# bupt-ai-cz/HIAST

Measured on AMD Instinct MI355X. Metric: self-training images/sec (fwd+bwd+pseudo-label) at 1024x512, higher is better.
Workload: dtype fp16

## Files before the change

hiast_amd/_lib.py:

```python
import ctypes
import os

import torch

_HERE = os.path.dirname(os.path.abspath(__file__))
LIB_PATH = os.environ.get("HIAST_LIB") or os.path.join(_HERE, "csrc", "libhiast_hip.so")

c_int, c_i64, c_f32, c_sz, c_vp = (ctypes.c_int, ctypes.c_int64, ctypes.c_float, ctypes.c_size_t,
                                   ctypes.c_void_p)

SIGNATURES = {
    "hiast_version": (c_int, []),
    "hiast_error_string": (ctypes.c_char_p, [c_int]),
    "hiast_upsample_bilinear_ac_fwd": (c_int, [c_vp, c_vp] + [c_int] * 6 + [c_vp]),
    "hiast_upsample_bilinear_ac_bwd": (c_int, [c_vp, c_vp] + [c_int] * 6 + [c_vp]),
    "hiast_plabel_pass1_workspace_bytes": (c_sz, [c_int]),
    "hiast_plabel_pass1": (c_int, [c_vp] + [c_int] * 6 + [c_vp, c_vp, c_vp, c_vp, c_sz, c_vp]),
    "hiast_plabel_pass2": (c_int, [c_vp, c_vp, c_vp, c_int, c_int, c_i64, c_vp, c_vp, c_vp, c_vp]),
    "hiast_plabel_strided_hist_workspace_bytes": (c_sz, [c_i64, c_int]),
    "hiast_plabel_strided_hist": (c_int, [c_vp, c_vp, c_i64, c_int, c_int, c_vp, c_vp, c_vp, c_vp, c_sz, c_vp]),
    "hiast_tta_fused": (c_int, [c_vp] * 6 + [c_int] * 5 + [c_vp, c_vp, c_vp]),
    "hiast_dinput_fwd": (c_int, [c_vp, c_int, c_vp] + [c_int] * 6 + [c_vp]),
    "hiast_dinput_bwd": (c_int, [c_vp, c_int, c_vp, c_vp, c_vp] + [c_int] * 6 + [c_vp]),
    "hiast_st_loss_workspace_bytes": (c_sz, [c_int] * 6),
# ... 30 lines not shown
    "hiast_stream_destroy": (c_int, [c_vp]),
    "hiast_igemm_stats_rows": (c_int, [c_i64, c_int, c_int, c_int, c_int]),
    "hiast_igemm_dgrad_bn_stats": (c_int, [c_vp, c_vp, c_vp] + [c_int] * 7 + [c_vp] * 6 + [c_int, c_int, c_vp]),
    "hiast_xconv_dgrad_gated_bn_stats_rows": (c_int, [c_i64, c_int, c_int]),
    "hiast_xconv_dgrad_gated_bn_stats": (c_int, [c_vp] * 10 + [c_i64, c_int, c_int, c_int, c_vp]),
    "hiast_igemm_dgrad_s2": (c_int, [c_vp, c_vp, c_vp] + [c_int] * 6 + [c_vp]),
    "hiast_igemm_dgrad_bn_stats_rows": (c_int, [c_i64, c_int, c_int, c_int]),
    "hiast_bn_nhwc_stats_from_partial": (c_int, [c_vp, c_int, c_int, c_vp, c_vp]),
    "hiast_conv_wgrad_workspace_bytes": (c_sz, [c_int] * 6),
    "hiast_conv_wgrad_nhwc": (c_int, [c_vp, c_vp, c_vp] + [c_int] * 9 + [c_vp, c_sz, c_vp]),
    "hiast_conv_wgrad_group_workspace_bytes": (c_sz, [c_vp, c_int]),
    "hiast_conv_wgrad_group_nhwc": (c_int, [c_vp, c_int, c_int, c_vp, c_sz, c_vp]),
    "hiast_conv_wgrad_small_workspace_bytes": (c_sz, [c_int] * 6),
    "hiast_conv_wgrad_small_nhwc": (c_int, [c_vp, c_vp, c_vp] + [c_int] * 9 + [c_vp, c_sz, c_vp]),
    "hiast_pack_conv_weight": (c_int, [c_vp, c_int, c_int, c_int, c_int, c_int, c_vp, c_vp, c_vp]),
    "hiast_bn_nhwc_workspace_bytes": (c_sz, [c_int]),
    "hiast_bn_nhwc_stats": (c_int, [c_vp, c_i64, c_int, c_vp, c_vp, c_sz, c_int, c_vp]),
    "hiast_bn_nhwc_apply": (c_int, [c_vp] * 8 + [ctypes.c_double, c_f32, c_f32, c_int, c_vp, c_vp, c_i64, c_int, c_vp,
                                    c_int, c_vp]),
    "hiast_bn_nhwc_apply_partial": (c_int, [c_vp] * 8 + [c_int, ctypes.c_double, c_f32, c_f32, c_int, c_vp, c_vp, c_i64,
                                            c_int, c_vp, c_int, c_vp]),
    "hiast_bn_nhwc_bwd_stats": (c_int, [c_vp] * 7 + [c_int, c_i64, c_int, c_vp, c_vp, c_sz, c_int, c_vp]),
    "hiast_bn_nhwc_bwd_apply": (c_int, [c_vp] * 8 + [ctypes.c_double, c_int, c_vp, c_vp, c_vp, c_vp, c_i64, c_int, c_int,
                                        c_vp]),
    "hiast_pack_conv_weight_multi": (c_int, [c_vp, c_vp, c_vp, c_int, c_int, c_vp]),
    "hiast_split_planes": (c_int, [c_vp, c_vp, c_i64, c_int, c_int, c_vp]),
    "hiast_stem_tail": (c_int, [c_vp, c_int, c_vp, c_vp, c_vp, c_vp, c_f32, c_vp, c_int, c_int, c_int, c_int, c_int, c_vp]),
    "hiast_stem_eval": (c_int, [c_vp] * 6 + [c_f32, c_vp, c_int, c_int, c_int, c_int, c_vp]),
    "hiast_stem_train_blocks": (c_int, [c_int] * 3),
    "hiast_stem_train_fwd": (c_int, [c_vp, c_vp, c_vp, c_vp, c_int, c_int, c_int, c_int, c_vp]),
    "hiast_stem_wgrad_workspace_bytes": (c_sz, [c_int] * 3),
    "hiast_stem_wgrad": (c_int, [c_vp, c_vp, c_vp, c_int, c_int, c_int, c_int, c_vp, c_sz, c_vp]),
    "hiast_ema_update": (c_int, [c_vp, c_vp, c_vp, c_int, c_f32, c_f32, c_vp]),
    "hiast_normalize_u8": (c_int, [c_vp, c_vp, c_int, c_i64, c_vp, c_vp, c_vp]),
    "hiast_maxpool3x3s2_nhwc_fwd": (c_int, [c_vp, c_vp, c_vp, c_int, c_int, c_int, c_int, c_int, c_vp]),
    "hiast_maxpool3x3s2_nhwc_bwd": (c_int, [c_vp, c_vp, c_vp, c_int, c_int, c_int, c_int, c_int, c_vp]),
    "hiast_multi_copy": (c_int, [c_vp, c_int, c_vp]),
    "hiast_aug_geometry_u8": (c_int, [c_vp] * 6 + [c_int] * 4 + [c_vp]),
    "hiast_aug_hist_u8": (c_int, [c_vp] * 5 + [c_int, c_i64, c_vp]),
    "hiast_aug_colour_u8": (c_int, [c_vp] * 5 + [c_int, c_i64, c_vp]),
    "hiast_aug2_table_u8": (c_int, [c_vp] * 6 + [c_int, c_i64, c_vp]),
    "hiast_aug2_colour_u8": (c_int, [c_vp] * 6 + [c_int, c_i64, c_vp]),
    "hiast_aug2_blur_u8": (c_int, [c_vp] * 5 + [c_int] * 3 + [c_vp]),
    "hiast_adam_prepare": (c_int, [c_vp, c_vp, c_vp, c_vp]),
    "hiast_adam_step": (c_int, [c_vp, c_vp, c_vp, c_int, ctypes.c_double, ctypes.c_double, c_f32, c_f32, c_vp, c_vp]),
    "hiast_disc_conv_workspace_bytes": (c_sz, [c_int] * 5),
    "hiast_disc_conv_fwd": (c_int, [c_vp] * 4 + [c_int] * 6 + [c_vp]),
    "hiast_disc_conv_dgrad": (c_int, [c_vp] * 4 + [c_int] * 6 + [c_vp, c_sz, c_vp]),
    "hiast_disc_conv_wgrad": (c_int, [c_vp] * 5 + [c_int] * 6 + [c_vp, c_sz, c_vp]),
    "hiast_confusion_hist": (c_int, [c_vp, c_vp, c_i64, c_int, c_vp, c_vp, c_vp, c_vp]),
}



class WgradJob(ctypes.Structure):
    _fields_ = [("dy", c_vp), ("x", c_vp), ("dw", c_vp)] + [(n, ctypes.c_int32) for n in
                                                             ("B", "H", "W", "Cin", "Cout", "taps", "stride", "dil")]


NBINS = 15361
PROB_FX_SHIFT = 30
IGNORE = 255

_lib = None


# ... 43 lines not shown
```

hiast_amd/csrc/igemm.hip:

```cpp
#include "igemm_kernel.h"

namespace hiast {

template <int PL>
__device__ __forceinline__ size_t ig_wp_elem(int n, int t, int k, int taps, int KO)
{
    const size_t row = ((size_t)n * taps + t) * PL * KO;
    return PL == 2 ? row + (size_t)(k >> 5) * 64 + (k & 31) : row + k;
}

template <int PL, bool F16 = false>
__global__ __launch_bounds__(256) void pack_conv_weight_kernel(const float* __restrict__ w,
                                                               unsigned short* __restrict__ wp,
                                                               unsigned short* __restrict__ wpt, int N, int K, int taps,
                                                               int mode)
{
    const long long idx = (long long)blockIdx.x * 256 + threadIdx.x;
    if (idx >= (long long)N * taps * K) return;
    const int k = (int)(idx % K);
    const int t = (int)((idx / K) % taps);
    const int n = (int)(idx / ((long long)K * taps));
    const float v = w[((size_t)n * K + k) * taps + t];
    unsigned short h, l = 0;
    if (F16) h = H16<true>::enc(v);
// ... 46 lines not shown
                if (PL == 2) *reinterpret_cast<uint4*>(d + 32) = *reinterpret_cast<const uint4*>(&lo[nt * PK_PITCH + c * 8]);
            }
        }
        if (adj) {
            for (int e = threadIdx.x; e < 64 * taps * (TN / 8); e += 256) {
                const int c = e % (TN / 8), kt = e / (TN / 8);
                const int k = kt / taps, t = kt - k * taps;
                unsigned short vh[8], vl[8];
#pragma unroll
                for (int j = 0; j < 8; ++j) {
                    vh[j] = hi[((c * 8 + j) * taps + t) * PK_PITCH + k];
                    if (PL == 2) vl[j] = lo[((c * 8 + j) * taps + t) * PK_PITCH + k];
                }
                unsigned short* d = adj + ig_wp_elem<PL>(k0 + k, taps - 1 - t, n0 + nh + c * 8, taps, N);
                *reinterpret_cast<uint4*>(d) = make_uint4(vh[0] | (unsigned)vh[1] << 16, vh[2] | (unsigned)vh[3] << 16,
                                                          vh[4] | (unsigned)vh[5] << 16, vh[6] | (unsigned)vh[7] << 16);
                if (PL == 2)
                    *reinterpret_cast<uint4*>(d + 32) = make_uint4(vl[0] | (unsigned)vl[1] << 16, vl[2] | (unsigned)vl[3] << 16,
                                                                   vl[4] | (unsigned)vl[5] << 16, vl[6] | (unsigned)vl[7] << 16);
            }
        }
    }
}

template <int PL, bool F16 = false>
__global__ __launch_bounds__(256) void pack_conv_weight_tiled_kernel(const float* __restrict__ w,
                                                                     unsigned short* __restrict__ wp,
                                                                     unsigned short* __restrict__ wpt, int N, int K,
                                                                     int taps, int mode)
{
    extern __shared__ __attribute__((aligned(16))) unsigned short lds[];
    const int kt = K / 64;
    pack_tile<PL, F16>(w, wp, wpt, N, K, taps, mode, (int)(blockIdx.x / kt) * 64, (int)(blockIdx.x % kt) * 64, lds);
}

__global__ __launch_bounds__(256) void pack_conv_weight_multi_kernel(const hiast_pack_rec* __restrict__ table,
                                                                     const int32_t* __restrict__ chunk_tensor,
                                                                     const int64_t* __restrict__ chunk_start)
{
    extern __shared__ __attribute__((aligned(16))) unsigned short lds[];
    const hiast_pack_rec r = table[chunk_tensor[blockIdx.x]];
    const int kt = r.K / 64;
    const int tile = (int)chunk_start[blockIdx.x];
    const int n0 = (tile / kt) * 64, k0 = (tile % kt) * 64;
    if (r.planes == HIAST_FMT_SPLIT_BF16)
        pack_tile<2>(r.w, (unsigned short*)r.wp, (unsigned short*)r.wpt, r.N, r.K, r.taps, r.mode, n0, k0, lds);
    else if (r.planes == HIAST_FMT_FP16)
        pack_tile<1, true>(r.w, (unsigned short*)r.wp, (unsigned short*)r.wpt, r.N, r.K, r.taps, r.mode, n0, k0, lds);
    else
        pack_tile<1>(r.w, (unsigned short*)r.wp, (unsigned short*)r.wpt, r.N, r.K, r.taps, r.mode, n0, k0, lds);
}

__global__ __launch_bounds__(256) void to_planes_kernel(const float* __restrict__ x, unsigned short* __restrict__ p,
                                                        long long M, int C)
{
    const long long total8 = M * C / 8;
    for (long long i = (long long)blockIdx.x * 256 + threadIdx.x; i < total8; i += (long long)gridDim.x * 256) {
        const long long m = (i * 8) / C;
        const int c = (int)((i * 8) - m * C);
        const float4 a = reinterpret_cast<const float4*>(x)[2 * i], b = reinterpret_cast<const float4*>(x)[2 * i + 1];
        const float v[8] = {a.x, a.y, a.z, a.w, b.x, b.y, b.z, b.w};
        unsigned ph[4], pl_[4];
#pragma unroll
        for (int q = 0; q < 4; ++q) {
            unsigned short h0, l0, h1, l1;
            ig_split(v[2 * q], h0, l0);
// ... 365 lines not shown
    else if (dtype == 1) { if (planes == 2) L(1, 2); else L(1, 1); }
    else { if (planes == 2) L(0, 2); else L(0, 1); }
#undef LF
#undef L
    HIAST_CHECK_LAUNCH();
    return 0;
}

extern "C" int hiast_split_planes(float* x, void* planes, int64_t M, int C, int inverse, hiast_stream_t stream)
{
    if (!x || !planes) return HIAST_E_ARG;
    if (M <= 0 || C <= 0) return HIAST_E_ARG;
    if (C % 32 != 0 || ((((uintptr_t)x) | ((uintptr_t)planes)) & 15)) return HIAST_E_RANGE;
    const long long total8 = (long long)M * C / 8;
    long long nb = (total8 + 255) / 256;
    const int grid = (int)(nb < 1 ? 1 : (nb > 8192 ? 8192 : nb));
    if (inverse)
        hipLaunchKernelGGL(hiast::from_planes_kernel, dim3(grid), dim3(256), 0, (hipStream_t)stream,
                           (const unsigned short*)planes, x, (long long)M, C);
    else
        hipLaunchKernelGGL(hiast::to_planes_kernel, dim3(grid), dim3(256), 0, (hipStream_t)stream, (const float*)x,
                           (unsigned short*)planes, (long long)M, C);
    HIAST_CHECK_LAUNCH();
    return 0;
}

extern "C" int hiast_pack_conv_weight_multi(const hiast_pack_rec* table, const int32_t* chunk_tensor,
                                            const int64_t* chunk_start, int n_chunks, int max_taps, hiast_stream_t stream)
{
    if (!table || !chunk_tensor || !chunk_start) return HIAST_E_ARG;
    if (n_chunks <= 0 || max_taps <= 0) return HIAST_E_ARG;
    if (max_taps > 9) return HIAST_E_RANGE;
    const size_t lds_bytes = (size_t)32 * max_taps * hiast::PK_PITCH * sizeof(unsigned short);
    hipLaunchKernelGGL(hiast::pack_conv_weight_multi_kernel, dim3(n_chunks), dim3(256), lds_bytes, (hipStream_t)stream, table,
                       chunk_tensor, chunk_start);
    HIAST_CHECK_LAUNCH();
    return 0;
}
```

hiast_amd/csrc/misc.hip:

```cpp
#include <hip/hip_bf16.h>

#include <atomic>

#include "common.h"

namespace hiast {

__global__ __launch_bounds__(256) void ema_kernel(const hiast_ema_rec* __restrict__ table,
                                                  const int32_t* __restrict__ chunk_tensor,
                                                  const int64_t* __restrict__ chunk_start,
                                                  float gamma, float omg)
{
    const hiast_ema_rec r = table[chunk_tensor[blockIdx.x]];
    const int64_t s = chunk_start[blockIdx.x];
    const int64_t e = (s + 65536 < r.n) ? s + 65536 : r.n;
    float* __restrict__ d = r.ema;
    const float* __restrict__ p = r.p;
    const bool vec = ((((uintptr_t)d) | ((uintptr_t)p)) & 15) == 0;
    if (vec) {
        const int64_t nv = (e - s) / 4;
        float4* d4 = reinterpret_cast<float4*>(d + s);
        const float4* p4 = reinterpret_cast<const float4*>(p + s);
        for (int64_t i = threadIdx.x; i < nv; i += 256) {
            float4 a = d4[i], b = p4[i];
            a.x = a.x * gamma + b.x * omg;
            a.y = a.y * gamma + b.y * omg;
            a.z = a.z * gamma + b.z * omg;
            a.w = a.w * gamma + b.w * omg;
            d4[i] = a;
        }
        for (int64_t i = s + nv * 4 + threadIdx.x; i < e; i += 256) d[i] = d[i] * gamma + p[i] * omg;
    } else {
        for (int64_t i = s + threadIdx.x; i < e; i += 256) d[i] = d[i] * gamma + p[i] * omg;
    }
}

__global__ __launch_bounds__(256) void normalize_u8_kernel(const unsigned char* __restrict__ img, float* __restrict__ out,
                                                           long long HW, float m0, float m1, float m2, float s0, float s1,
                                                           float s2)
{
    const int b = blockIdx.y;
    const unsigned char* src = img + (size_t)b * HW * 3;
    float* dst = out + (size_t)b * 3 * HW;
    for (long long p = (long long)blockIdx.x * 256 + threadIdx.x; p < HW; p += (long long)gridDim.x * 256) {
        const float r = (float)src[p * 3] / 255.0f, g = (float)src[p * 3 + 1] / 255.0f, bl = (float)src[p * 3 + 2] / 255.0f;
        dst[p] = (r - m0) / s0;
        dst[HW + p] = (g - m1) / s1;
        dst[2 * HW + p] = (bl - m2) / s2;
    }
}

__global__ __launch_bounds__(256) void multi_copy_kernel(const hiast_copy_rec* __restrict__ table)
{
    const hiast_copy_rec r = table[blockIdx.x];
    unsigned char* d = (unsigned char*)r.dst;
    const unsigned char* s = (const unsigned char*)r.src;
    if (((((uintptr_t)d) | ((uintptr_t)s)) & 15) == 0) {
        const int64_t nv = r.nbytes / 16;
        for (int64_t i = threadIdx.x; i < nv; i += 256) reinterpret_cast<uint4*>(d)[i] = reinterpret_cast<const uint4*>(s)[i];
        for (int64_t i = nv * 16 + threadIdx.x; i < r.nbytes; i += 256) d[i] = s[i];
    } else {
        for (int64_t i = threadIdx.x; i < r.nbytes; i += 256) d[i] = s[i];
    }
}

__global__ void adam_prepare_kernel(hiast_adam_ctl* __restrict__ ctl, const float* __restrict__ grad_scale,
                                    const float* __restrict__ found_inf)
// ... 148 lines not shown
    return 0;
}
extern "C" int hiast_stream_destroy(hiast_stream_t s)
{
    if (!s) return HIAST_E_ARG;
    const hipError_t e = hipStreamDestroy((hipStream_t)s);
    if (e != hipSuccess) { (void)hipGetLastError(); return (int)e; }
    return 0;
}

extern "C" const char* hiast_error_string(int code)
{
    switch (code) {
        case 0: return "ok";
        case HIAST_E_ARG: return "hiast: null pointer or non-positive extent";
        case HIAST_E_RANGE: return "hiast: extent outside the range the kernels are built for";
        case HIAST_E_WS: return "hiast: workspace too small";
        default: return code > 0 ? hipGetErrorString((hipError_t)code) : "hiast: unknown error";
    }
}

extern "C" int hiast_ema_update(const hiast_ema_rec* table, const int32_t* chunk_tensor,
                                const int64_t* chunk_start, int n_chunks, float gamma,
                                float one_minus_gamma, hiast_stream_t stream)
{
    if (!table || !chunk_tensor || !chunk_start) return HIAST_E_ARG;
    if (n_chunks <= 0) return HIAST_E_ARG;
    hipLaunchKernelGGL(hiast::ema_kernel, dim3(n_chunks), dim3(256), 0, (hipStream_t)stream, table,
                       chunk_tensor, chunk_start, gamma, one_minus_gamma);
    HIAST_CHECK_LAUNCH();
    return 0;
}

extern "C" int hiast_confusion_hist(const int64_t* pred, const int64_t* target, int64_t N, int K,
                                    int64_t* inter, int64_t* area_pred, int64_t* area_tgt,
                                    hiast_stream_t stream)
{
    if (!pred || !target || !inter || !area_pred || !area_tgt) return HIAST_E_ARG;
    if (N <= 0 || K <= 0) return HIAST_E_ARG;
    if (K > 1024) return HIAST_E_RANGE;
    int64_t nb = (N + 256 * 16 - 1) / (256 * 16);
    int grid = (int)(nb < 1 ? 1 : (nb > 2048 ? 2048 : nb));
    hipLaunchKernelGGL(hiast::confusion_kernel, dim3(grid), dim3(256), 3 * K * sizeof(unsigned),
                       (hipStream_t)stream, pred, target, N, K, (unsigned long long*)inter,
                       (unsigned long long*)area_pred, (unsigned long long*)area_tgt);
    HIAST_CHECK_LAUNCH();
    return 0;
}

extern "C" int hiast_adam_step(const hiast_adam_rec* table, const int32_t* chunk_tensor, const int64_t* chunk_start,
                               int n_chunks, double beta1, double beta2, float eps, float weight_decay,
                               const hiast_adam_ctl* ctl, hiast_stream_t stream)
{
    if (!table || !chunk_tensor || !chunk_start) return HIAST_E_ARG;
    if (n_chunks <= 0) return HIAST_E_ARG;
    hipLaunchKernelGGL(hiast::adam_kernel, dim3(n_chunks), dim3(256), 0, (hipStream_t)stream, table, chunk_tensor,
                       chunk_start, (float)beta1, (float)beta2, (float)(1.0 - beta1), (float)(1.0 - beta2), eps,
                       weight_decay, ctl, beta1, beta2);
    HIAST_CHECK_LAUNCH();
    return 0;
}

extern "C" int hiast_adam_prepare(hiast_adam_ctl* ctl, const float* grad_scale, const float* found_inf,
                                  hiast_stream_t stream)
{
    if (!ctl) return HIAST_E_ARG;
// ... 170 lines not shown
```

hiast_amd/kernels.py:

```python
import ctypes

import numpy as np
import torch

from . import _lib
from . import switches as _SW
from ._lib import NBINS, check


def _stream():
    return ctypes.c_void_p(torch._C._cuda_getCurrentRawStream(torch._C._cuda_getDevice()))


def _ptr(t):
    return ctypes.c_void_p(t.data_ptr()) if t is not None else ctypes.c_void_p(0)


def h2d_async(host, device, out=None):
    stage = torch.from_numpy(np.ascontiguousarray(host)).pin_memory()
    if out is None:
        return stage.to(device, non_blocking=True)
    out.copy_(stage.view(out.dtype).reshape(out.shape) if stage.dtype != out.dtype else stage.reshape(out.shape),
              non_blocking=True)
    return out
# ... 485 lines not shown
    def __init__(self, ema_tensors, src_tensors):
        assert len(ema_tensors) == len(src_tensors) and len(ema_tensors) > 0
        dev = ema_tensors[0].device
        recs = np.zeros((len(ema_tensors), 3), dtype=np.int64)
        ct, cs = [], []
        for i, (e, p) in enumerate(zip(ema_tensors, src_tensors)):
            _req(e, torch.float32, None, "ema tensor")
            _req(p, torch.float32, None, "student tensor")
            assert e.numel() == p.numel()
            recs[i] = (e.data_ptr(), p.data_ptr(), e.numel())
            for s in range(0, e.numel(), self.CHUNK):
                ct.append(i)
                cs.append(s)
        self.keep = (list(ema_tensors), list(src_tensors))
        self.table = torch.from_numpy(recs).to(dev)
        self.chunk_tensor = torch.tensor(ct, dtype=torch.int32, device=dev)
        self.chunk_start = torch.tensor(cs, dtype=torch.int64, device=dev)
        self.n_chunks = len(ct)
        self.ptrs = recs[:, :2].copy()

    def still_valid(self):
        return all(e.data_ptr() == a and p.data_ptr() == b
                   for (e, p, (a, b)) in zip(self.keep[0], self.keep[1], self.ptrs))

    def matches(self, ema_tensors, src_tensors):
        return len(ema_tensors) == len(self.ptrs) and all(
            e.data_ptr() == a and p.data_ptr() == b for (e, p, (a, b)) in zip(ema_tensors, src_tensors, self.ptrs))


def ema_update(plan, gamma):
    check(_lib.load().hiast_ema_update(_ptr(plan.table), _ptr(plan.chunk_tensor), _ptr(plan.chunk_start),
                                       plan.n_chunks, float(np.float32(gamma)), float(np.float32(1 - gamma)),
                                       _stream()), "hiast_ema_update")


def normalize_u8(img_u8, mean, std):
    _req(img_u8, torch.uint8, 4, "img_u8")
    B, H, W, three = img_u8.shape
    assert three == 3 and len(mean) == 3 and len(std) == 3
    out = torch.empty((B, 3, H, W), dtype=torch.float32, device=img_u8.device)
    m = (ctypes.c_float * 3)(*[float(v) for v in mean])
    s_ = (ctypes.c_float * 3)(*[float(v) for v in std])
    if B:
        check(_lib.load().hiast_normalize_u8(_ptr(img_u8), _ptr(out), B, H * W, m, s_, _stream()), "hiast_normalize_u8")
    return out


class CopyPlan:

    def __init__(self, dsts, srcs):
        assert len(dsts) == len(srcs) and len(dsts) > 0
        recs = np.zeros((len(dsts), 3), dtype=np.int64)
        for i, (d, s_) in enumerate(zip(dsts, srcs)):
            if not (d.is_cuda and s_.is_cuda and d.is_contiguous() and s_.is_contiguous() and d.dtype == s_.dtype
                    and d.numel() == s_.numel()):
                raise ValueError("multi_copy: tensor %d: contiguous HIP tensors of equal dtype and size required" % i)
            recs[i] = (d.data_ptr(), s_.data_ptr(), d.numel() * d.element_size())
        self.keep = (list(dsts), list(srcs))
        self.ptrs = recs[:, :2].copy()
        self.table = torch.from_numpy(recs).to(dsts[0].device)
        self.n = len(dsts)

    def still_valid(self):
        return all(d.data_ptr() == a and s_.data_ptr() == b for (d, s_, (a, b)) in zip(self.keep[0], self.keep[1], self.ptrs))

    def matches(self, dsts, srcs):
# ... 476 lines not shown
    M, C2 = p.shape
    x = torch.empty((M, C2 // 2), dtype=torch.float32, device=p.device)
    check(_lib.load().hiast_split_planes(_ptr(x), _ptr(p), M, C2 // 2, 1, _stream()), "hiast_split_planes")
    return x


def pack_conv_weight(weight, fmt, transpose=False, both=False):
    fmt = int(fmt)
    planes, h16 = (2 if fmt == FMT_SPLIT_BF16 else 1), fmt_dtype(fmt)
    w = weight.detach()
    if w.dim() == 2:
        w = w.reshape(w.shape[0], w.shape[1], 1, 1)
    _req(w, torch.float32, 4, "weight")
    N, K_, kh, kw = w.shape
    fwd_shape, adj_shape = (N, kh * kw, planes * K_), (K_, kh * kw, planes * N)
    wpt = None
    if both:
        wp = torch.empty(fwd_shape, dtype=h16, device=w.device)
        wpt = torch.empty(adj_shape, dtype=h16, device=w.device)
        mode = 2
    else:
        wp = torch.empty(adj_shape if transpose else fwd_shape, dtype=h16, device=w.device)
        mode = 1 if transpose else 0
    check(_lib.load().hiast_pack_conv_weight(_ptr(w), N, K_, kh * kw, fmt, mode, _ptr(wp), _ptr(wpt), _stream()),
          "hiast_pack_conv_weight")
    return (wp, wpt) if both else wp


class PackPlan:
    CHUNK = 65536
    REC = np.dtype([("w", np.int64), ("wp", np.int64), ("wpt", np.int64), ("N", np.int32), ("K", np.int32),
                    ("taps", np.int32), ("planes", np.int32), ("mode", np.int32), ("pad", np.int32)])

    def __init__(self, weights, fmt, adjoint):
        assert len(weights) > 0 and len(weights) == len(adjoint)
        dev = weights[0].device
        fmt = int(fmt)
        planes, h16 = (2 if fmt == FMT_SPLIT_BF16 else 1), fmt_dtype(fmt)
        self.weights, self.fmt = list(weights), fmt
        self.wp, self.wpt = [], []
        host = np.zeros(len(weights), dtype=self.REC)
        lists = {}
        for i, (w, adj) in enumerate(zip(weights, adjoint)):
            _req(w.detach(), torch.float32, 4, "weight")
            N, K_, kh, kw = w.shape
            taps = kh * kw
            wp = torch.empty((N, taps, planes * K_), dtype=h16, device=dev)
            wpt = torch.empty((K_, taps, planes * N), dtype=h16, device=dev) if adj else None
            self.wp.append(wp)
            self.wpt.append(wpt)
            host[i] = (w.data_ptr(), wp.data_ptr(), wpt.data_ptr() if adj else 0, N, K_, taps, fmt, 2 if adj else 0, 0)
            if N % 64 or K_ % 64 or taps > 9:
                raise ValueError("PackPlan: channel counts must be multiples of 64 (got %d x %d)" % (N, K_))
            ct, cs = lists.setdefault(taps, ([], []))
            for tile in range((N // 64) * (K_ // 64)):
                ct.append(i)
                cs.append(tile)
        self.ptrs = [w.data_ptr() for w in weights]
        self.table = torch.from_numpy(host.view(np.uint8).reshape(-1).copy()).to(dev)
        self.launches = [(taps, torch.tensor(ct, dtype=torch.int32, device=dev), torch.tensor(cs, dtype=torch.int64, device=dev),
                          len(ct)) for taps, (ct, cs) in sorted(lists.items())]
        self.versions = None

    def still_valid(self):
        return all(w.data_ptr() == p for w, p in zip(self.weights, self.ptrs))

    def refresh(self):
        v = [w._version for w in self.weights]
        if v == self.versions:
            return False
        for taps, ct, cs, n in self.launches:
            check(_lib.load().hiast_pack_conv_weight_multi(_ptr(self.table), _ptr(ct), _ptr(cs), n, taps, _stream()),
                  "hiast_pack_conv_weight_multi")
        self.versions = v
        return True


def igemm_bn_act(x, wp, planes, bn, res, relu, stride=1, dil=1, out_f32=False, want_stats=False, res_gate=None):
    _req16(x, 4, "x")
    PL = 2 if int(planes) == 2 else 1
    fmt = fmt_of(x, PL)
# ... 393 lines not shown
```

hiast_amd/workflows/trainer/base_trainer.py:

```python
import os

import numpy as np
import torch
import torch.distributed as dist

from hiast_amd import functional as HF
from torch.nn.parallel import DistributedDataParallel as DDP
from torch.utils.data import DataLoader, DistributedSampler

from hiast_amd.sseg.datasets import utils as du
from hiast_amd.utils import comm, metrics, utils
from hiast_amd.utils.registry.registries import DATASET
from hiast_amd.utils.result_recorder import ResultRecorder


def autocast_dtype(cfg):
    if cfg.train.apex_opt == "O0":
        return None
    kind = getattr(cfg.train, "amp_dtype", "fp16")
    if kind not in ("bf16", "fp16"):
        raise ValueError("train.amp_dtype must be 'bf16' or 'fp16', got %r" % (kind,))
    return torch.bfloat16 if kind == "bf16" else torch.float16


def make_grad_scaler(amp_dtype):
    if amp_dtype is torch.float16:
        return torch.amp.GradScaler("cuda", init_scale=2.0 ** 16, growth_factor=2.0, backoff_factor=0.5, growth_interval=2000)
    return None


def _worker_init(_worker_id):
    try:
        os.nice(10)
    except OSError:
        pass


class _EpochChain(torch.utils.data.Sampler):

    def __init__(self, sampler, batch_size, drop_last):
        self.sampler, self.batch_size, self.drop_last = sampler, batch_size, drop_last

    def __iter__(self):
        while True:
            n = 0
            for b in torch.utils.data.BatchSampler(self.sampler, self.batch_size, self.drop_last):
                n += 1
                yield b
            if n == 0:
                return
            self.sampler.set_epoch(self.sampler.epoch + 1)

    def __len__(self):
        return len(torch.utils.data.BatchSampler(self.sampler, self.batch_size, self.drop_last))


class _Bare(torch.nn.Module):

    def __init__(self, m):
        super().__init__()
# ... 240 lines not shown
```

include/hiast_hip.h:

```cpp
#ifndef HIAST_HIP_H
#define HIAST_HIP_H

#include <stddef.h>
#include <stdint.h>

#ifdef __cplusplus
extern "C" {
#endif

#define HIAST_ABI_VERSION 6

#define HIAST_E_ARG   (-1)
#define HIAST_E_RANGE (-2)
#define HIAST_E_WS    (-3)

#define HIAST_NBINS 15361
#define HIAST_PROB_FX_SHIFT 30
#define HIAST_MAX_CLASSES 32
#define HIAST_FMT_BF16 1
#define HIAST_FMT_SPLIT_BF16 2
#define HIAST_FMT_FP16 3
#define HIAST_IGNORE 255

typedef void* hiast_stream_t;
// ... 145 lines not shown
size_t hiast_conv_wgrad_group_workspace_bytes(const hiast_wgrad_job* jobs, int njobs);
int hiast_conv_wgrad_group_nhwc(const hiast_wgrad_job* jobs, int njobs, int fmt, void* workspace, size_t workspace_bytes,
                                hiast_stream_t stream);

size_t hiast_conv_wgrad_small_workspace_bytes(int B, int H, int W, int Cin, int Cout, int taps);
int hiast_conv_wgrad_small_nhwc(const void* dy, const void* x, float* dw, int B, int H, int W, int Cin, int Cout, int taps,
                                int stride, int dil, int fmt, void* workspace, size_t workspace_bytes, hiast_stream_t stream);

size_t hiast_bn_nhwc_workspace_bytes(int C);
int hiast_bn_nhwc_stats(const void* x, int64_t M, int C, double* sums, void* workspace, size_t workspace_bytes, int fmt,
                        hiast_stream_t stream);
int hiast_bn_nhwc_stats_from_partial(const float* partial, int nblk, int C, double* sums, hiast_stream_t stream);
int hiast_bn_nhwc_apply_partial(const void* x, const void* res, void* y, const float* gamma, const float* beta,
                                float* running_mean, float* running_var, const float* partial, int nblk, double count,
                                float momentum, float eps, int relu, float* save_mean, float* save_invstd, int64_t M,
                                int C, void* mask, int fmt, hiast_stream_t stream);
int hiast_bn_nhwc_apply(const void* x, const void* res, void* y, const float* gamma, const float* beta,
                        float* running_mean, float* running_var, const double* sums, double count, float momentum,
                        float eps, int relu, float* save_mean, float* save_invstd, int64_t M, int C, void* mask, int fmt,
                        hiast_stream_t stream);
int hiast_bn_nhwc_bwd_stats(const void* dy, const void* y, const void* x, const float* gamma, const float* beta,
                            const float* save_mean, const float* save_invstd, int relu, int64_t M, int C, double* sums,
                            void* workspace, size_t workspace_bytes, int fmt, hiast_stream_t stream);
int hiast_bn_nhwc_bwd_apply(const void* dy, const void* y, const void* x, const float* gamma, const float* beta,
                            const float* save_mean, const float* save_invstd, const double* sums, double count, int relu,
                            void* dx, void* dres, float* dgamma, float* dbeta, int64_t M, int C, int fmt,
                            hiast_stream_t stream);

typedef struct { float* ema; const float* p; int64_t n; } hiast_ema_rec;
int hiast_ema_update(const hiast_ema_rec* table, const int32_t* chunk_tensor,
                     const int64_t* chunk_start, int n_chunks, float gamma,
                     float one_minus_gamma, hiast_stream_t stream);

int hiast_maxpool3x3s2_nhwc_fwd(const void* x, void* y, uint8_t* idx, int B, int H, int W, int C,
                                int fmt , hiast_stream_t stream);
int hiast_maxpool3x3s2_nhwc_bwd(const void* dy, const uint8_t* idx, void* dx, int B, int H, int W, int C, int fmt,
                                hiast_stream_t stream);

int hiast_normalize_u8(const uint8_t* img, float* out, int B, int64_t HW, const float* mean, const float* std,
                       hiast_stream_t stream);

#define HIAST_AUG_REC_WORDS 20
#define HIAST_AUG_MAX_OPS 8
#define HIAST_AUG_OPS_WORDS (4 + 2 * HIAST_AUG_MAX_OPS)
#define HIAST_AUG_OP_LUT 1
#define HIAST_AUG_OP_GRAY 2
#define HIAST_AUG_OP_EQUALIZE 3
int hiast_aug_geometry_u8(const int64_t* recs, const uint8_t* blob, const int32_t* tabs, uint8_t* tmp,
                          uint8_t* img_out, uint8_t* lbl_out, int B, int max_ch, int oh, int ow, hiast_stream_t stream);
int hiast_aug_hist_u8(const int64_t* ops, const uint8_t* blob, const uint8_t* in, uint32_t* hist, uint8_t* eq_lut,
                      int B, int64_t HW, hiast_stream_t stream);
int hiast_aug_colour_u8(const int64_t* ops, const uint8_t* blob, const uint8_t* eq_lut, const uint8_t* in,
                        uint8_t* out, int B, int64_t HW, hiast_stream_t stream);

#define HIAST_AUG_OP_CONTRAST 4
#define HIAST_AUG_OP_SAT 5
#define HIAST_AUG_OP_HUE 6
#define HIAST_AUG_OP_BLUR 7
#define HIAST_AUG_MAX_KSIZE 41
int hiast_aug2_table_u8(const int64_t* ops, const int32_t* seg, const uint8_t* blob, const uint8_t* in, uint32_t* hist,
                        uint8_t* table, int B, int64_t HW, hiast_stream_t stream);
int hiast_aug2_colour_u8(const int64_t* ops, const int32_t* seg, const uint8_t* blob, const uint8_t* table,
                         const uint8_t* in, uint8_t* out, int B, int64_t HW, hiast_stream_t stream);
int hiast_aug2_blur_u8(const int64_t* ops, const int32_t* seg, const int32_t* tabs, uint8_t* img, float* tmp, int B,
                       int H, int W, hiast_stream_t stream);

// ... 32 lines not shown
```

Before: 143.9.

## Add read-only grad non-finite check and specialised weight-pack kernels

Replaces GradScaler's per-device inf check with a custom multi-tensor kernel that only reads gradients and sets a flag, instead of a check that also rewrites every gradient. Adds specialised weight-packing kernels: a 1x1 kernel that walks several chunks per block and prefetches the next chunk's weights, and a 3x3 kernel that splits each tile across two blocks using vectorised float4 loads. PackPlan can also write into preallocated output tensors. This adds a host-side table upload per step and a larger kernel surface.

```diff
diff --git a/hiast_amd/_lib.py b/hiast_amd/_lib.py
--- a/hiast_amd/_lib.py
+++ b/hiast_amd/_lib.py
@@ -86,6 +86,7 @@
     "hiast_stem_wgrad_workspace_bytes": (c_sz, [c_int] * 3),
     "hiast_stem_wgrad": (c_int, [c_vp, c_vp, c_vp, c_int, c_int, c_int, c_int, c_vp, c_sz, c_vp]),
     "hiast_ema_update": (c_int, [c_vp, c_vp, c_vp, c_int, c_f32, c_f32, c_vp]),
+    "hiast_grads_nonfinite": (c_int, [c_vp, c_vp, c_vp, c_int, c_vp, c_vp]),
     "hiast_normalize_u8": (c_int, [c_vp, c_vp, c_int, c_i64, c_vp, c_vp, c_vp]),
     "hiast_maxpool3x3s2_nhwc_fwd": (c_int, [c_vp, c_vp, c_vp, c_int, c_int, c_int, c_int, c_int, c_vp]),
     "hiast_maxpool3x3s2_nhwc_bwd": (c_int, [c_vp, c_vp, c_vp, c_int, c_int, c_int, c_int, c_int, c_vp]),
diff --git a/hiast_amd/csrc/igemm.hip b/hiast_amd/csrc/igemm.hip
--- a/hiast_amd/csrc/igemm.hip
+++ b/hiast_amd/csrc/igemm.hip
@@ -102,6 +102,166 @@
     extern __shared__ __attribute__((aligned(16))) unsigned short lds[];
     const int kt = K / 64;
     pack_tile<PL, F16>(w, wp, wpt, N, K, taps, mode, (int)(blockIdx.x / kt) * 64, (int)(blockIdx.x % kt) * 64, lds);
+}
+
+template <int TAPS, int TN>
+struct PkPass {
+    static constexpr int RUN4 = 16 * TAPS;
+    static constexpr int NV = TN * RUN4 / 256;
+    static_assert(TN * RUN4 % 256 == 0, "a pass must fill whole rounds of the block");
+};
+
+template <int TAPS, int TN>
+__device__ __forceinline__ void pk_fetch(const float* __restrict__ w, int K, int nb, int k0,
+                                         float4 (&v)[PkPass<TAPS, TN>::NV])
+{
+    using P = PkPass<TAPS, TN>;
+    const bool vec = (((uintptr_t)w) & 15) == 0;
+#pragma unroll
+    for (int i = 0; i < P::NV; ++i) {
+        const int e4 = threadIdx.x + i * 256;
+        const int n = e4 / P::RUN4, r = (e4 - n * P::RUN4) * 4;
+        const float* s = w + ((size_t)(nb + n) * K + k0) * TAPS + r;
+        if (vec) v[i] = *reinterpret_cast<const float4*>(s);
+        else v[i] = make_float4(s[0], s[1], s[2], s[3]);
+    }
+}
+
+template <int TAPS, int PL, bool F16, int TN>
+__device__ __forceinline__ void pk_emit(const float4 (&v)[PkPass<TAPS, TN>::NV], unsigned short* __restrict__ wp,
+                                        unsigned short* __restrict__ wpt, int N, int K, int mode, int nb, int k0,
+                                        unsigned short* lds)
+{
+    using P = PkPass<TAPS, TN>;
+    unsigned short* hi = lds;
+    unsigned short* lo = lds + (PL == 2 ? TN * TAPS * PK_PITCH : 0);
+    unsigned short* fwd = (mode == 1) ? nullptr : wp;
+    unsigned short* adj = (mode == 0) ? nullptr : (mode == 1 ? wp : wpt);
+#pragma unroll
+    for (int i = 0; i < P::NV; ++i) {
+        const int e4 = threadIdx.x + i * 256;
+        const int n = e4 / P::RUN4, r = (e4 - n * P::RUN4) * 4;
+        const float f[4] = {v[i].x, v[i].y, v[i].z, v[i].w};
+#pragma unroll
+        for (int j = 0; j < 4; ++j) {
+            const int k = (r + j) / TAPS, t = (r + j) - k * TAPS;
+            unsigned short h, l = 0;
+            if (F16) h = H16<true>::enc(f[j]);
+            else ig_split(f[j], h, l);
+            hi[(n * TAPS + t) * PK_PITCH + k] = h;
+            if (PL == 2) lo[(n * TAPS + t) * PK_PITCH + k] = l;
+        }
+    }
+    __syncthreads();
+    if (fwd) {
+        for (int e = threadIdx.x; e < TN * TAPS * 8; e += 256) {
+            const int c = e & 7, nt = e >> 3;
+            const int n = nt / TAPS, t = nt - n * TAPS;
+            unsigned short* d = fwd + ig_wp_elem<PL>(nb + n, t, k0 + c * 8, TAPS, K);
+            *reinterpret_cast<uint4*>(d) = *reinterpret_cast<const uint4*>(&hi[nt * PK_PITCH + c * 8]);
+            if (PL == 2) *reinterpret_cast<uint4*>(d + 32) = *reinterpret_cast<const uint4*>(&lo[nt * PK_PITCH + c * 8]);
+        }
+    }
+    if (adj) {
+        for (int e = threadIdx.x; e < 64 * TAPS * (TN / 8); e += 256) {
+            const int c = e % (TN / 8), kt = e / (TN / 8);
+            const int k = kt / TAPS, t = kt - k * TAPS;
+            unsigned short vh[8], vl[8];
+#pragma unroll
+            for (int j = 0; j < 8; ++j) {
+                vh[j] = hi[((c * 8 + j) * TAPS + t) * PK_PITCH + k];
+                if (PL == 2) vl[j] = lo[((c * 8 + j) * TAPS + t) * PK_PITCH + k];
+            }
+            unsigned short* d = adj + ig_wp_elem<PL>(k0 + k, TAPS - 1 - t, nb + c * 8, TAPS, N);
+            *reinterpret_cast<uint4*>(d) = make_uint4(vh[0] | (unsigned)vh[1] << 16, vh[2] | (unsigned)vh[3] << 16,
+                                                      vh[4] | (unsigned)vh[5] << 16, vh[6] | (unsigned)vh[7] << 16);
+            if (PL == 2)
+                *reinterpret_cast<uint4*>(d + 32) = make_uint4(vl[0] | (unsigned)vl[1] << 16, vl[2] | (unsigned)vl[3] << 16,
+                                                               vl[4] | (unsigned)vl[5] << 16, vl[6] | (unsigned)vl[7] << 16);
+        }
+    }
+    __syncthreads();
+}
+
+template <int TAPS, int TN>
+__device__ __forceinline__ void pk_emit_fmt(const float4 (&v)[PkPass<TAPS, TN>::NV], const hiast_pack_rec& r, int nb, int k0,
+                                            unsigned short* lds)
+{
+    if (r.planes == HIAST_FMT_FP16)
+        pk_emit<TAPS, 1, true, TN>(v, (unsigned short*)r.wp, (unsigned short*)r.wpt, r.N, r.K, r.mode, nb, k0, lds);
+    else
+        pk_emit<TAPS, 1, false, TN>(v, (unsigned short*)r.wp, (unsigned short*)r.wpt, r.N, r.K, r.mode, nb, k0, lds);
+}
+
+__global__ __launch_bounds__(256) void pack_conv_weight_multi9_kernel(const hiast_pack_rec* __restrict__ table,
+                                                                      const int32_t* __restrict__ chunk_tensor,
+                                                                      const int64_t* __restrict__ chunk_start)
+{
+    extern __shared__ __attribute__((aligned(16))) unsigned short lds[];
+    const int chunk = blockIdx.x >> 1, half = blockIdx.x & 1;
+    const hiast_pack_rec r = table[chunk_tensor[chunk]];
+    const int kt = r.K / 64;
+    const int tile = (int)chunk_start[chunk];
+    const int n0 = (tile / kt) * 64, k0 = (tile % kt) * 64;
+    if (r.taps != 9) {
+        if (half) return;
+        if (r.planes == HIAST_FMT_SPLIT_BF16)
+            pack_tile<2>(r.w, (unsigned short*)r.wp, (unsigned short*)r.wpt, r.N, r.K, r.taps, r.mode, n0, k0, lds);
+        else if (r.planes == HIAST_FMT_FP16)
+            pack_tile<1, true>(r.w, (unsigned short*)r.wp, (unsigned short*)r.wpt, r.N, r.K, r.taps, r.mode, n0, k0, lds);
+        else
+            pack_tile<1>(r.w, (unsigned short*)r.wp, (unsigned short*)r.wpt, r.N, r.K, r.taps, r.mode, n0, k0, lds);
+        return;
+    }
+    const int nb = n0 + half * 32;
+    if (r.planes == HIAST_FMT_SPLIT_BF16) {
+        float4 a[PkPass<9, 16>::NV], b[PkPass<9, 16>::NV];
+        pk_fetch<9, 16>(r.w, r.K, nb, k0, a);
+        pk_fetch<9, 16>(r.w, r.K, nb + 16, k0, b);
+        pk_emit<9, 2, false, 16>(a, (unsigned short*)r.wp, (unsigned short*)r.wpt, r.N, r.K, r.mode, nb, k0, lds);
+        pk_emit<9, 2, false, 16>(b, (unsigned short*)r.wp, (unsigned short*)r.wpt, r.N, r.K, r.mode, nb + 16, k0, lds);
+    } else {
+        float4 a[PkPass<9, 32>::NV];
+        pk_fetch<9, 32>(r.w, r.K, nb, k0, a);
+        pk_emit_fmt<9, 32>(a, r, nb, k0, lds);
+    }
+}
+
+constexpr int PK_WALK = 4;
+
+__global__ __launch_bounds__(256) void pack_conv_weight_multi1_kernel(const hiast_pack_rec* __restrict__ table,
+                                                                      const int32_t* __restrict__ chunk_tensor,
+                                                                      const int64_t* __restrict__ chunk_start, int n_chunks)
+{
+    extern __shared__ __attribute__((aligned(16))) unsigned short lds[];
+    const int first = blockIdx.x * PK_WALK;
+    const int last = first + PK_WALK < n_chunks ? first + PK_WALK : n_chunks;
+    if (first >= last) return;
+    hiast_pack_rec r = table[chunk_tensor[first]];
+    int tile = (int)chunk_start[first];
+    int n0 = (tile / (r.K / 64)) * 64, k0 = (tile % (r.K / 64)) * 64;
+    float4 v[PkPass<1, 64>::NV], vn[PkPass<1, 64>::NV];
+    pk_fetch<1, 64>(r.w, r.K, n0, k0, v);
+    for (int c = first; c < last; ++c) {
+        hiast_pack_rec rn = r;
+        int n0n = 0, k0n = 0;
+        if (c + 1 < last) {
+            rn = table[chunk_tensor[c + 1]];
+            tile = (int)chunk_start[c + 1];
+            n0n = (tile / (rn.K / 64)) * 64;
+            k0n = (tile % (rn.K / 64)) * 64;
+            pk_fetch<1, 64>(rn.w, rn.K, n0n, k0n, vn);
+        }
+        if (r.planes == HIAST_FMT_SPLIT_BF16)
+            pk_emit<1, 2, false, 64>(v, (unsigned short*)r.wp, (unsigned short*)r.wpt, r.N, r.K, r.mode, n0, k0, lds);
+        else
+            pk_emit_fmt<1, 64>(v, r, n0, k0, lds);
+#pragma unroll
+        for (int i = 0; i < PkPass<1, 64>::NV; ++i) v[i] = vn[i];
+        r = rn;
+        n0 = n0n;
+        k0 = k0n;
+    }
 }
 
 __global__ __launch_bounds__(256) void pack_conv_weight_multi_kernel(const hiast_pack_rec* __restrict__ table,
@@ -533,6 +693,20 @@
     if (n_chunks <= 0 || max_taps <= 0) return HIAST_E_ARG;
     if (max_taps > 9) return HIAST_E_RANGE;
     const size_t lds_bytes = (size_t)32 * max_taps * hiast::PK_PITCH * sizeof(unsigned short);
+    if (max_taps == 1 && n_chunks < (1 << 30)) {
+        const int grid = (n_chunks + hiast::PK_WALK - 1) / hiast::PK_WALK;
+        hipLaunchKernelGGL(hiast::pack_conv_weight_multi1_kernel, dim3(grid), dim3(256),
+                           (size_t)2 * 64 * hiast::PK_PITCH * sizeof(unsigned short), (hipStream_t)stream, table,
+                           chunk_tensor, chunk_start, n_chunks);
+        HIAST_CHECK_LAUNCH();
+        return 0;
+    }
+    if (max_taps == 9 && n_chunks < (1 << 30)) {
+        hipLaunchKernelGGL(hiast::pack_conv_weight_multi9_kernel, dim3(2u * (unsigned)n_chunks), dim3(256), lds_bytes,
+                           (hipStream_t)stream, table, chunk_tensor, chunk_start);
+        HIAST_CHECK_LAUNCH();
+        return 0;
+    }
     hipLaunchKernelGGL(hiast::pack_conv_weight_multi_kernel, dim3(n_chunks), dim3(256), lds_bytes, (hipStream_t)stream, table,
                        chunk_tensor, chunk_start);
     HIAST_CHECK_LAUNCH();
diff --git a/hiast_amd/csrc/misc.hip b/hiast_amd/csrc/misc.hip
--- a/hiast_amd/csrc/misc.hip
+++ b/hiast_amd/csrc/misc.hip
@@ -33,6 +33,37 @@
     } else {
         for (int64_t i = s + threadIdx.x; i < e; i += 256) d[i] = d[i] * gamma + p[i] * omg;
     }
+}
+
+__global__ __launch_bounds__(256) void grads_nonfinite_kernel(const hiast_grad_rec* __restrict__ table,
+                                                              const int32_t* __restrict__ chunk_tensor,
+                                                              const int64_t* __restrict__ chunk_start,
+                                                              float* __restrict__ found_inf)
+{
+    const hiast_grad_rec r = table[chunk_tensor[blockIdx.x]];
+    const int64_t s = chunk_start[blockIdx.x];
+    const int64_t e = (s + 65536 < r.n) ? s + 65536 : r.n;
+    const float* __restrict__ g = r.g;
+    auto bad1 = [](float x) -> unsigned { return (__float_as_uint(x) & 0x7F800000u) == 0x7F800000u ? 1u : 0u; };
+    unsigned bad = 0;
+    if ((((uintptr_t)g) & 15) == 0) {
+        const int64_t nv = (e - s) / 4;
+        const float4* g4 = reinterpret_cast<const float4*>(g + s);
+        int64_t i = threadIdx.x;
+        for (; i + 768 < nv; i += 1024) {
+            const float4 a = g4[i], b = g4[i + 256], c = g4[i + 512], d = g4[i + 768];
+            bad |= bad1(a.x) | bad1(a.y) | bad1(a.z) | bad1(a.w) | bad1(b.x) | bad1(b.y) | bad1(b.z) | bad1(b.w) |
+                   bad1(c.x) | bad1(c.y) | bad1(c.z) | bad1(c.w) | bad1(d.x) | bad1(d.y) | bad1(d.z) | bad1(d.w);
+        }
+        for (; i < nv; i += 256) {
+            const float4 a = g4[i];
+            bad |= bad1(a.x) | bad1(a.y) | bad1(a.z) | bad1(a.w);
+        }
+        for (int64_t j = s + nv * 4 + threadIdx.x; j < e; j += 256) bad |= bad1(g[j]);
+    } else {
+        for (int64_t j = s + threadIdx.x; j < e; j += 256) bad |= bad1(g[j]);
+    }
+    if (bad) found_inf[0] = 1.0f;
 }
 
 __global__ __launch_bounds__(256) void normalize_u8_kernel(const unsigned char* __restrict__ img, float* __restrict__ out,
@@ -247,6 +278,17 @@
     return 0;
 }
 
+extern "C" int hiast_grads_nonfinite(const hiast_grad_rec* table, const int32_t* chunk_tensor, const int64_t* chunk_start,
+                                     int n_chunks, float* found_inf, hiast_stream_t stream)
+{
+    if (!table || !chunk_tensor || !chunk_start || !found_inf) return HIAST_E_ARG;
+    if (n_chunks <= 0) return HIAST_E_ARG;
+    hipLaunchKernelGGL(hiast::grads_nonfinite_kernel, dim3(n_chunks), dim3(256), 0, (hipStream_t)stream, table,
+                       chunk_tensor, chunk_start, found_inf);
+    HIAST_CHECK_LAUNCH();
+    return 0;
+}
+
 extern "C" int hiast_confusion_hist(const int64_t* pred, const int64_t* target, int64_t N, int K,
                                     int64_t* inter, int64_t* area_pred, int64_t* area_tgt,
                                     hiast_stream_t stream)
diff --git a/hiast_amd/kernels.py b/hiast_amd/kernels.py
--- a/hiast_amd/kernels.py
+++ b/hiast_amd/kernels.py
@@ -541,6 +541,52 @@
     check(_lib.load().hiast_ema_update(_ptr(plan.table), _ptr(plan.chunk_tensor), _ptr(plan.chunk_start),
                                        plan.n_chunks, float(np.float32(gamma)), float(np.float32(1 - gamma)),
                                        _stream()), "hiast_ema_update")
+
+
+class NonfinitePlan:
+    CHUNK = 65536
+
+    def __init__(self, numels, device):
+        ct, cs = [], []
+        for i, n in enumerate(numels):
+            for s0 in range(0, n, self.CHUNK):
+                ct.append(i)
+                cs.append(s0)
+        self.numels = tuple(numels)
+        self.chunk_tensor = torch.tensor(ct, dtype=torch.int32, device=device)
+        self.chunk_start = torch.tensor(cs, dtype=torch.int64, device=device)
+        self.n_chunks = len(ct)
+        self.host = np.zeros((len(numels), 2), dtype=np.int64)
+        self.table = torch.empty((len(numels), 2), dtype=torch.int64, device=device)
+
+
+_nonfinite_plans = {}
+
+
+def grads_nonfinite(grads, found_inf):
+    if not (isinstance(found_inf, torch.Tensor) and found_inf.is_cuda and found_inf.dtype == torch.float32
+            and found_inf.numel() == 1):
+        raise ValueError("grads_nonfinite: found_inf must be a float32 device scalar")
+    grads = [g for g in grads if g.numel()]
+    for i, g in enumerate(grads):
+        if not (g.is_cuda and g.dtype == torch.float32 and g.is_contiguous() and g.device == found_inf.device):
+            raise ValueError("grads_nonfinite: gradient %d must be a contiguous float32 tensor on %s" % (i, found_inf.device))
+    if not grads:
+        return found_inf
+    key = (found_inf.device, tuple(g.numel() for g in grads))
+    plan = _nonfinite_plans.get(key)
+    if plan is None:
+        if len(_nonfinite_plans) >= 8:
+            _nonfinite_plans.clear()
+        plan = _nonfinite_plans[key] = NonfinitePlan(key[1], found_inf.device)
+    h = plan.host
+    for i, g in enumerate(grads):
+        h[i, 0] = g.data_ptr()
+        h[i, 1] = g.numel()
+    h2d_async(h, plan.table.device, out=plan.table)
+    check(_lib.load().hiast_grads_nonfinite(_ptr(plan.table), _ptr(plan.chunk_tensor), _ptr(plan.chunk_start),
+                                            plan.n_chunks, _ptr(found_inf), _stream()), "hiast_grads_nonfinite")
+    return found_inf
 
 
 def normalize_u8(img_u8, mean, std):
@@ -1083,8 +1129,9 @@
     REC = np.dtype([("w", np.int64), ("wp", np.int64), ("wpt", np.int64), ("N", np.int32), ("K", np.int32),
                     ("taps", np.int32), ("planes", np.int32), ("mode", np.int32), ("pad", np.int32)])
 
-    def __init__(self, weights, fmt, adjoint):
+    def __init__(self, weights, fmt, adjoint, out=None):
         assert len(weights) > 0 and len(weights) == len(adjoint)
+        assert out is None or len(out) == len(weights)
         dev = weights[0].device
         fmt = int(fmt)
         planes, h16 = (2 if fmt == FMT_SPLIT_BF16 else 1), fmt_dtype(fmt)
@@ -1096,8 +1143,19 @@
             _req(w.detach(), torch.float32, 4, "weight")
             N, K_, kh, kw = w.shape
             taps = kh * kw
-            wp = torch.empty((N, taps, planes * K_), dtype=h16, device=dev)
-            wpt = torch.empty((K_, taps, planes * N), dtype=h16, device=dev) if adj else None
+            if out is None:
+                wp = torch.empty((N, taps, planes * K_), dtype=h16, device=dev)
+                wpt = torch.empty((K_, taps, planes * N), dtype=h16, device=dev) if adj else None
+            else:
+                wp, wpt = out[i]
+                wpt = wpt if adj else None
+                for t, shape, nm in ((wp, (N, taps, planes * K_), "wp"), (wpt, (K_, taps, planes * N), "wpt")):
+                    if nm == "wpt" and not adj:
+                        continue
+                    _req(t, h16, 3, "out[%d].%s" % (i, nm))
+                    if tuple(t.shape) != shape or t.device != dev or t.data_ptr() % 16:
+                        raise ValueError("PackPlan: out[%d].%s must be a 16-byte aligned %s tensor on %s, got %s"
+                                         % (i, nm, shape, dev, tuple(t.shape)))
             self.wp.append(wp)
             self.wpt.append(wpt)
             host[i] = (w.data_ptr(), wp.data_ptr(), wpt.data_ptr() if adj else 0, N, K_, taps, fmt, 2 if adj else 0, 0)
diff --git a/hiast_amd/workflows/trainer/base_trainer.py b/hiast_amd/workflows/trainer/base_trainer.py
--- a/hiast_amd/workflows/trainer/base_trainer.py
+++ b/hiast_amd/workflows/trainer/base_trainer.py
@@ -23,9 +23,28 @@
     return torch.bfloat16 if kind == "bf16" else torch.float16
 
 
+class _ReadOnlyCheckScaler(torch.amp.GradScaler):
+
+    def _check_inf_per_device(self, optimizer):
+        _scale, _ = self._check_scale_growth_tracker("_check_inf_per_device")
+        grads = [p.grad for group in optimizer.param_groups for p in group["params"] if p.grad is not None]
+        dev = _scale.device
+        if not grads or dev.type != "cuda" or not all(
+                g.device == dev and g.dtype == torch.float32 and g.layout == torch.strided and g.is_contiguous()
+                for g in grads):
+            return super()._check_inf_per_device(optimizer)
+        from hiast_amd import kernels as K
+        found_inf = torch.full((), 0.0, dtype=torch.float32, device=dev)
+        with torch.no_grad():
+            K.grads_nonfinite(grads, found_inf)
+        self._per_optimizer_states[id(optimizer)]["found_inf_per_device"] = {dev: found_inf}
+        return self._per_optimizer_states[id(optimizer)]["found_inf_per_device"]
+
+
 def make_grad_scaler(amp_dtype):
     if amp_dtype is torch.float16:
-        return torch.amp.GradScaler("cuda", init_scale=2.0 ** 16, growth_factor=2.0, backoff_factor=0.5, growth_interval=2000)
+        return _ReadOnlyCheckScaler("cuda", init_scale=2.0 ** 16, growth_factor=2.0, backoff_factor=0.5,
+                                    growth_interval=2000)
     return None
 
 
diff --git a/include/hiast_hip.h b/include/hiast_hip.h
--- a/include/hiast_hip.h
+++ b/include/hiast_hip.h
@@ -201,6 +201,10 @@
                      const int64_t* chunk_start, int n_chunks, float gamma,
                      float one_minus_gamma, hiast_stream_t stream);
 
+typedef struct { const float* g; int64_t n; } hiast_grad_rec;
+int hiast_grads_nonfinite(const hiast_grad_rec* table, const int32_t* chunk_tensor, const int64_t* chunk_start,
+                          int n_chunks, float* found_inf, hiast_stream_t stream);
+
 int hiast_maxpool3x3s2_nhwc_fwd(const void* x, void* y, uint8_t* idx, int B, int H, int W, int C,
                                 int fmt , hiast_stream_t stream);
 int hiast_maxpool3x3s2_nhwc_bwd(const void* dy, const uint8_t* idx, void* dx, int B, int H, int W, int C, int fmt,
```

Measured after the change: 144.7 (median of 6 runs). No clear change (+0.6%).
